# kawshik8/GAN-Image-Captioning

Measured on AMD Instinct MI355X. Metric: captions/sec (G+D train step), higher is better.
Workload: dtype bf16; 1 GPU; cfg2: adversarial G+D step, batch 64/GPU, 224x224 images, caption len 20, V=10000, E=H=512, 1-layer LSTM G, CNN-seq D (R=64,F=900), ResNet-50-shaped encoder, --conditional-gan 1; global_batch=64, caption_len=20, image_size=224, vocab=10000, conditional_gan=1, encoder=resnet50, step_impl=fused, parallelism=dp1

## Files before the change

gan-image-captioning_amd/csrc/gemm.hip:

```cpp
#include "gemm.h"
#include "conv3x3.h"
#include "conv1x1_stream.h"
#include "conv1x1_panel.h"
#include "conv1x1_pix.h"
#include "conv_stem.h"
#include "bn_fold.h"
#include "kernels.h"

#include <stdlib.h>

namespace gic {

namespace {

typedef __attribute__((address_space(3))) bf16x4 lds_bf16x4;
typedef unsigned int u32x4 __attribute__((ext_vector_type(4)));
typedef const __attribute__((address_space(1))) u32x4* gptr_u4;

__device__ __attribute__((aligned(16))) unsigned int g_zero16[4] = {0u, 0u, 0u, 0u};
typedef __attribute__((address_space(3))) void* lds_void_ptr;
typedef const __attribute__((address_space(1))) void* gbl_void_ptr;

#ifdef GIC_STAMPS
}
// ... 404 lines not shown
    for (int j = 0; j < TN; ++j) {
      const int n = bn0 + wc * (BN / 2) + j * 16 + lr;
      if (n >= N) continue;
      const float bias = (d.bias && blockIdx.y == 0) ? d.bias[n] : 0.f;
      const int mb = bm0 + wr * (BM / 2) + i * 16 + lg * 4;
      float keep4[4] = {1.f, 1.f, 1.f, 1.f};
      if constexpr (EPI == EPI_HIGHWAY) {
        if (!d.mask && d.use_philox) {
          uint32_t r0, r1, r2, r3;
          Philox::gen4(d.seed_dev ? *d.seed_dev : d.seed, d.stream, (uint64_t)(mb >> 2) * (uint64_t)N + (uint64_t)n, r0, r1, r2, r3);
          keep4[0] = Philox::u01(r0) >= d.drop_p ? 1.f : 0.f;
          keep4[1] = Philox::u01(r1) >= d.drop_p ? 1.f : 0.f;
          keep4[2] = Philox::u01(r2) >= d.drop_p ? 1.f : 0.f;
          keep4[3] = Philox::u01(r3) >= d.drop_p ? 1.f : 0.f;
        }
      }
      float st_s = 0.f, st_q = 0.f;
#pragma unroll
      for (int r = 0; r < 4; ++r) {
        const int m = mb + r;
        if (m >= M) continue;
        float v = d.alpha * acc[i][j][r] + bias;
        if constexpr (EPI == EPI_BNSTATS) {
          C[(long)m * d.ldc + n] = from_f32<TO>(v);
          st_s += v; st_q += v * v;
        } else if constexpr (EPI == EPI_PLAIN) {
          const long o = (long)m * d.ldc + n;
          if constexpr (sizeof(TO) == 4) {
            if (split) { atomicAdd((float*)&C[o], v); continue; }
          }
          if (d.accumulate) v += to_f32<TO>(C[o]);
          C[o] = from_f32<TO>(v);
        } else {
          const float x = to_f32<TI>(((const TI*)d.X)[(long)m * d.ldx + n]);
          const float sg = 1.f / (1.f + expf(-v));
          const float y = sg * fmaxf(v, 0.f) + (1.f - sg) * x;
          if (d.Hpre) d.Hpre[(long)m * d.ldh + n] = v;
          float keep = keep4[r];
          if (d.mask) keep = (float)d.mask[(long)m * d.ldmask + n];
          if (d.mask_out) d.mask_out[(long)m * d.ldmask_out + n] = (uint8_t)keep;
          C[(long)m * d.ldc + n] = from_f32<TO>(y * keep * d.keep_scale);
        }
      }
      if constexpr (EPI == EPI_BNSTATS) {
        st_s += __shfl_xor(st_s, 16, 64); st_q += __shfl_xor(st_q, 16, 64);
        st_s += __shfl_xor(st_s, 32, 64); st_q += __shfl_xor(st_q, 32, 64);
        float* st = d.stats + (long)(blockIdx.x % d.stats_nrep) * 2 * N;
        if (lg == 0) { atomicAdd(&st[n], st_s); atomicAdd(&st[N + n], st_q); }
      }
    }
  }
}

template <typename TO, int BN, int EPI, bool CONV, int NS, bool ABN = false, bool ARES = false, int AMAXK = (ARES ? 2048 : 1024)>
__global__ __launch_bounds__(512) void tile8_kernel(const GemmDesc d, const unsigned a_bytes, const unsigned b_bytes) {
  static_assert(!ARES || ABN, "the residual-on-load form extends the A-side BatchNorm");
  constexpr int BM = 128, BK = 64, NT = 512;
  constexpr int TM = 2, TN = BN / 32;
  constexpr int CA = BM * 8 / NT, CB = BN * 8 / NT;
  constexpr int NL = CA + CB + (ARES ? CA : 0);
  constexpr int A_BYTES = BM * 128, B_BYTES = BN * 128, R_BYTES = ARES ? A_BYTES : 0, STAGE = A_BYTES + B_BYTES + R_BYTES;
  constexpr int OSZ = sizeof(TO), OVE = 16 / OSZ, SC = BN * OSZ + 16;
  constexpr int EPI_BYTES = EPI == EPI_HIGHWAY ? BM * (BN + 4) * 4 : (EPI == EPI_GUMBELMAX ? 8 * BN * 4 : BM * SC + 8 * (BN / 2) * 2 * 4);
  constexpr int RING_BYTES = NS * STAGE > EPI_BYTES ? NS * STAGE : EPI_BYTES;
  constexpr int ABN_MAXK = AMAXK;
  constexpr int SMEM_BYTES = RING_BYTES + (ABN ? ABN_MAXK * 8 : 0) + (ARES ? ABN_MAXK * 8 : 0);
  constexpr unsigned OOB = 0x80000000u;
  static_assert(CB >= 1 && SMEM_BYTES <= 160 * 1024, "tile8 LDS budget");
  __shared__ __attribute__((aligned(16))) unsigned char smem[SMEM_BYTES];

  const int tid = threadIdx.x, lane = tid & 63, w = tid >> 6;
  STAMP(0);
  const int wr = w >> 1, wc = w & 1;
  const int lr = lane & 15, lg = lane >> 4;

  const int tiles_m = (d.M + BM - 1) / BM, tiles_n = (d.N + BN - 1) / BN;
  const int bid = xcd_run(blockIdx.x, gridDim.x);
  const int bm0 = (d.n_fast ? bid / tiles_n : bid % tiles_m) * BM;
  const int bn0 = (d.n_fast ? bid % tiles_n : bid / tiles_m) * BN;
  const int M = d.M, N = d.N, K = d.K;

  const __amdgpu_buffer_rsrc_t rsA = __builtin_amdgcn_make_buffer_rsrc((void*)d.A, 0, (int)a_bytes, 0x00020000);
  const __amdgpu_buffer_rsrc_t rsB = __builtin_amdgcn_make_buffer_rsrc((void*)d.B, 0, (int)b_bytes, 0x00020000);
  const __amdgpu_buffer_rsrc_t rsR = __builtin_amdgcn_make_buffer_rsrc((void*)(ARES ? d.res : d.A), 0, (int)a_bytes, 0x00020000);

  const int kc = ((tid & 7) ^ ((tid >> 4) & 7)) * 8;
  int a_off[CA], a_hi0[CA], a_wi0[CA];
  bool a_ok[CA];
  int cv_r = 0, cv_s = 0, cv_c = 0;
#pragma unroll
  for (int i = 0; i < CA; ++i) {
    const int m = bm0 + (tid >> 3) + i * 64;
    a_ok[i] = m < M;
    if constexpr (CONV) {
      const int mm = a_ok[i] ? m : 0;
      const int wo = mm % d.cWo, t = mm / d.cWo;
      const int ho = t % d.cHo, n = t / d.cHo;
      a_hi0[i] = a_ok[i] ? ho * d.cStride - d.cPad : -(1 << 28);
      a_wi0[i] = wo * d.cStride - d.cPad;
      a_off[i] = ((n * d.cH + a_hi0[i]) * d.cW + a_wi0[i]) * d.cCin;
    } else {
      a_hi0[i] = a_wi0[i] = 0;
      a_off[i] = m * (int)d.lda;
    }
  }
  if constexpr (CONV) {
    cv_c = kc % d.cCin;
    const int t = kc / d.cCin;
    cv_s = t % d.cKW;
    cv_r = t / d.cKW;
  }
  int b_off[CB];
  bool b_ok[CB];
#pragma unroll
  for (int i = 0; i < CB; ++i) {
    const int n = bn0 + (tid >> 3) + i * 64;
    b_ok[i] = n < N;
    b_off[i] = n * (int)d.ldb;
  }
  const int wbase = (tid & ~63) * 16;

  auto issue = [&](int kt, int st) {
    unsigned char* sA = smem + st * STAGE;
    unsigned char* sB = sA + A_BYTES;
    const int k = kt * BK + kc;
    const bool kok = k < K;
#pragma unroll
    for (int i = 0; i < CA; ++i) {
      unsigned voff;
      if constexpr (CONV) {
        const bool ok = (unsigned)(a_hi0[i] + cv_r) < (unsigned)d.cH & (unsigned)(a_wi0[i] + cv_s) < (unsigned)d.cW & kok;
        voff = ok ? (unsigned)(a_off[i] + (cv_r * d.cW + cv_s) * d.cCin + cv_c) * 2u : OOB;
      } else {
        voff = (a_ok[i] & kok) ? (unsigned)(a_off[i] + k) * 2u : OOB;
      }
      __builtin_amdgcn_raw_ptr_buffer_load_lds(rsA, (lds_void_ptr)(sA + i * (NT * 16) + wbase), 16, (int)voff, 0, 0, CONV ? GIC_TRUNK_NT : 0);
      if constexpr (ARES)
        __builtin_amdgcn_raw_ptr_buffer_load_lds(rsR, (lds_void_ptr)(sB + B_BYTES + i * (NT * 16) + wbase), 16, (int)voff, 0, 0, CONV ? GIC_TRUNK_NT : 0);
    }
#pragma unroll
    for (int i = 0; i < CB; ++i) {
      const unsigned voff = (b_ok[i] & kok) ? (unsigned)(b_off[i] + k) * 2u : OOB;
      __builtin_amdgcn_raw_ptr_buffer_load_lds(rsB, (lds_void_ptr)(sB + i * (NT * 16) + wbase), 16, (int)voff, 0, 0, 0);
    }
    if constexpr (CONV) {
      cv_c += BK;
      while (cv_c >= d.cCin) {
        cv_c -= d.cCin;
        if (++cv_s == d.cKW) { cv_s = 0; ++cv_r; }
      }
    }
  };

  float* coef = (float*)(smem + RING_BYTES);
  if constexpr (ABN) {
    const int Cn = CONV ? d.cCin : K;
    for (int c = tid; c < ABN_MAXK; c += NT) {
      float sc = 0.f, sh = 0.f;
      if (c < Cn) {
        float s1, s2;
        fold_replicas(d.in_stats, d.in_nrep, Cn, c, s1, s2);
        const float mean = s1 * d.in_inv_count;
        const float var = fmaxf(s2 * d.in_inv_count - mean * mean, 0.f);
        sc = d.in_gamma[c] * rsqrtf(var + 1e-5f);
        sh = d.in_beta[c] - mean * sc;
      }
      coef[2 * c] = sc; coef[2 * c + 1] = sh;
      if constexpr (ARES) {
        float rs = 1.f, rt = 0.f;
        if (d.res_stats && c < Cn) {
          float s1, s2;
          fold_replicas(d.res_stats, d.res_nrep, Cn, c, s1, s2);
          const float mean = s1 * d.res_inv_count;
          const float var = fmaxf(s2 * d.res_inv_count - mean * mean, 0.f);
          rs = d.res_gamma[c] * rsqrtf(var + 1e-5f);
          rt = d.res_beta[c] - mean * rs;
        }
        coef[2 * ABN_MAXK + 2 * c] = rs; coef[2 * ABN_MAXK + 2 * c + 1] = rt;
      }
    }
    __syncthreads();
  }
  const bool wb = ARES && d.out_wb && bn0 == 0;
  auto abn = [&](int kt, int st) {
    if constexpr (ABN) {
      const int k = kt * BK + kc;
      if (k < K) {
        const int ch = CONV ? k % d.cCin : k;
        const int tap = CONV ? k / d.cCin : 0;
        const int ts = tap % (CONV ? d.cKW : 1), tr = tap / (CONV ? d.cKW : 1);
        const float4* cp = (const float4*)(coef + 2 * ch);
        const float4 c0 = cp[0], c1 = cp[1], c2 = cp[2], c3 = cp[3];
        const float scl[8] = {c0.x, c0.z, c1.x, c1.z, c2.x, c2.z, c3.x, c3.z};
        const float sft[8] = {c0.y, c0.w, c1.y, c1.w, c2.y, c2.w, c3.y, c3.w};
        float rsc[8] = {1.f, 1.f, 1.f, 1.f, 1.f, 1.f, 1.f, 1.f}, rsf[8] = {0.f, 0.f, 0.f, 0.f, 0.f, 0.f, 0.f, 0.f};
        if constexpr (ARES) {
          const float4* rp = (const float4*)(coef + 2 * ABN_MAXK + 2 * ch);
          const float4 r0 = rp[0], r1 = rp[1], r2 = rp[2], r3 = rp[3];
          rsc[0] = r0.x; rsc[1] = r0.z; rsc[2] = r1.x; rsc[3] = r1.z; rsc[4] = r2.x; rsc[5] = r2.z; rsc[6] = r3.x; rsc[7] = r3.z;
          rsf[0] = r0.y; rsf[1] = r0.w; rsf[2] = r1.y; rsf[3] = r1.w; rsf[4] = r2.y; rsf[5] = r2.w; rsf[6] = r3.y; rsf[7] = r3.w;
        }
#pragma unroll
        for (int i = 0; i < CA; ++i) {
          const bool ok = CONV ? ((unsigned)(a_hi0[i] + tr) < (unsigned)d.cH & (unsigned)(a_wi0[i] + ts) < (unsigned)d.cW) : a_ok[i];
          if (!ok) continue;
          bf16x8* p = (bf16x8*)(smem + st * STAGE + i * (NT * 16) + tid * 16);
          bf16x8 v = *p;
          if constexpr (ARES) {
            const bf16x8 r = *(const bf16x8*)(smem + st * STAGE + A_BYTES + B_BYTES + i * (NT * 16) + tid * 16);
#pragma unroll
            for (int e = 0; e < 8; ++e) v[e] = (bf16_t)fmaxf((float)v[e] * scl[e] + sft[e] + ((float)r[e] * rsc[e] + rsf[e]), 0.f);
            if (wb) *(bf16x8*)((bf16_t*)d.out_wb + (long)a_off[i] + k) = v;
          } else {
#pragma unroll
            for (int e = 0; e < 8; ++e) v[e] = (bf16_t)fmaxf((float)v[e] * scl[e] + sft[e], 0.f);
          }
          *p = v;
        }
      }
    }
  };

  f32x4 acc[TM][TN];
#pragma unroll
  for (int i = 0; i < TM; ++i)
#pragma unroll
    for (int j = 0; j < TN; ++j) acc[i][j] = (f32x4){0.f, 0.f, 0.f, 0.f};

  auto compute = [&](int st) {
    const unsigned char* sA = smem + st * STAGE;
    const unsigned char* sB = sA + A_BYTES;
    bf16x8 fa[2][TM], fb[2][TN];
#pragma unroll
    for (int ks = 0; ks < 2; ++ks) {
#pragma unroll
      for (int t = 0; t < TM; ++t) {
        const int row = wr * 32 + t * 16 + lr;
        fa[ks][t] = *(const bf16x8*)(sA + row * 128 + (((ks * 4 + lg) ^ ((row >> 1) & 7)) << 4));
      }
#pragma unroll
      for (int t = 0; t < TN; ++t) {
        const int row = wc * (BN / 2) + t * 16 + lr;
        fb[ks][t] = *(const bf16x8*)(sB + row * 128 + (((ks * 4 + lg) ^ ((row >> 1) & 7)) << 4));
      }
    }
#pragma unroll
    for (int ks = 0; ks < 2; ++ks)
#pragma unroll
      for (int i = 0; i < TM; ++i)
#pragma unroll
        for (int j = 0; j < TN; ++j)
          acc[i][j] = __builtin_amdgcn_mfma_f32_16x16x32_bf16(fa[ks][i], fb[ks][j], acc[i][j], 0, 0, 0);
  };

  auto read_half = [&](int st, int ks, bf16x8 (&fa)[TM], bf16x8 (&fb)[TN]) {
    const unsigned char* sA = smem + st * STAGE;
    const unsigned char* sB = sA + A_BYTES;
#pragma unroll
    for (int t = 0; t < TM; ++t) {
      const int row = wr * 32 + t * 16 + lr;
      fa[t] = *(const bf16x8*)(sA + row * 128 + (((ks * 4 + lg) ^ ((row >> 1) & 7)) << 4));
    }
#pragma unroll
    for (int t = 0; t < TN; ++t) {
      const int row = wc * (BN / 2) + t * 16 + lr;
      fb[t] = *(const bf16x8*)(sB + row * 128 + (((ks * 4 + lg) ^ ((row >> 1) & 7)) << 4));
    }
  };
  auto mfma_half = [&](const bf16x8 (&fa)[TM], const bf16x8 (&fb)[TN]) {
#pragma unroll
    for (int i = 0; i < TM; ++i)
#pragma unroll
      for (int j = 0; j < TN; ++j)
        acc[i][j] = __builtin_amdgcn_mfma_f32_16x16x32_bf16(fa[i], fb[j], acc[i][j], 0, 0, 0);
  };

  const int nk = (K + BK - 1) / BK;
  STAMP(1);
  if constexpr (NS == 1) {
    for (int kt = 0; kt < nk; ++kt) {
      if (kt) __builtin_amdgcn_s_barrier();
      issue(kt, 0);
      asm volatile("s_waitcnt vmcnt(0)" ::: "memory");
      abn(kt, 0);
      __builtin_amdgcn_s_barrier();
      compute(0);
    }
  } else if constexpr (NS < 4) {
    issue(0, 0);
    int st = 0;
    for (int kt = 0; kt < nk; ++kt) {
      asm volatile("s_waitcnt vmcnt(0)" ::: "memory");
      abn(kt, st);
      __builtin_amdgcn_s_barrier();
      if (kt == 0) STAMP(2);
      if (!(DBG & 1)) issue(kt + 1, st ^ 1);
      if (!(DBG & 2)) compute(st);
      st ^= 1;
    }
  } else {
#pragma unroll
    for (int s = 0; s < NS - 1; ++s) issue(s, s);
    bf16x8 fa0[TM], fb0[TN], fa1[TM], fb1[TN];
    int st = 0, st_fill = NS - 1;
    for (int kt = 0; kt < nk; ++kt) {
      asm volatile("s_waitcnt vmcnt(%0) lgkmcnt(0)" ::"n"(NS >= 2 ? (NS - 2) * NL : 0) : "memory");
      abn(kt, st);
      __builtin_amdgcn_s_barrier();
      if (kt == 0) STAMP(2);
      if (!(DBG & 2)) {
        read_half(st, 0, fa0, fb0);
        __builtin_amdgcn_sched_barrier(0);
        if (kt > 0) mfma_half(fa1, fb1);
        __builtin_amdgcn_sched_barrier(0);
      }
      if (!(DBG & 1)) issue(kt + NS - 1, st_fill);
      if (!(DBG & 2)) {
        __builtin_amdgcn_sched_barrier(0);
        read_half(st, 1, fa1, fb1);
        __builtin_amdgcn_sched_barrier(0);
        mfma_half(fa0, fb0);
      }
      st = st == NS - 1 ? 0 : st + 1;
      st_fill = st_fill == NS - 1 ? 0 : st_fill + 1;
    }
    if (!(DBG & 2) && nk > 0) mfma_half(fa1, fb1);
  }
  asm volatile("s_waitcnt vmcnt(0)" ::: "memory");
  __syncthreads();
  STAMP(3);

  if constexpr (EPI == EPI_GUMBELMAX) {
    float* sV = (float*)smem;
    int* sI = (int*)(smem + 4 * BN * 4);
    const float eps = 1e-10f;
    const uint64_t seed = d.seed_dev ? *d.seed_dev : d.seed;
    const float T = d.gm_temperature;
#pragma unroll
    for (int j = 0; j < TN; ++j) {
      const int nl = wc * (BN / 2) + j * 16 + lr;
      const int n = bn0 + nl;
      float best = -INFINITY;
      int best_i = 0x7fffffff;
#pragma unroll
      for (int i = 0; i < TM; ++i) {
        const int m0 = bm0 + wr * 32 + i * 16 + lg * 4;
        if (m0 < M && n < N) {
          const float4 bv = *(const float4*)(d.gm_bias + m0);
          const float bia[4] = {bv.x, bv.y, bv.z, bv.w};
          float uu[4];
          if (d.gm_u) {
            const float4 uv = *(const float4*)(d.gm_u + (long)n * d.gm_ldu + m0);
            uu[0] = uv.x; uu[1] = uv.y; uu[2] = uv.z; uu[3] = uv.w;
          } else {
            uint32_t r0, r1, r2, r3;
            Philox::gen4(seed, d.stream, (uint64_t)n * (uint64_t)(M >> 2) + (uint64_t)(m0 >> 2), r0, r1, r2, r3);
            uu[0] = Philox::u01(r0); uu[1] = Philox::u01(r1); uu[2] = Philox::u01(r2); uu[3] = Philox::u01(r3);
          }
#pragma unroll
          for (int r = 0; r < 4; ++r) {
            const float g = -__logf(-__logf(uu[r] + eps) + eps);
            const float y = (acc[i][j][r] + bia[r] + g) * T;
            if (y > best) { best = y; best_i = m0 + r; }
          }
        }
      }
#pragma unroll
      for (int o = 16; o <= 32; o <<= 1) {
        const float ob = __shfl_xor(best, o, 64);
        const int oi = __shfl_xor(best_i, o, 64);
        if (ob > best || (ob == best && oi < best_i)) { best = ob; best_i = oi; }
      }
      if (lg == 0) { sV[wr * BN + nl] = best; sI[wr * BN + nl] = best_i; }
    }
    __syncthreads();
    if (tid < BN && bn0 + tid < N) {
      float best = sV[tid];
      int best_i = sI[tid];
#pragma unroll
// ... 61 lines not shown
            if (d.mask && live) k = (float)d.mask[(long)m * d.ldmask + n0 + e];
            kb |= (unsigned long long)(live ? (unsigned)k : 0u) << (8 * e);
            yv[e] = (bf16_t)(live ? y * k * d.keep_scale : 0.f);
          }
          if (d.Hpre) {
            *(float4*)(d.Hpre + (long)m * d.ldh + n0) = h0;
            *(float4*)(d.Hpre + (long)m * d.ldh + n0 + 4) = h1;
          }
          if (d.mask_out) *(unsigned long long*)(d.mask_out + (long)m * d.ldmask_out + n0) = kb;
          *(bf16x8*)((bf16_t*)C + (long)m * d.ldc + n0) = yv;
        }
      }
      STAMP(5);
      return;
    }
#pragma unroll
    for (int i = 0; i < TM; ++i) {
#pragma unroll
      for (int j = 0; j < TN; ++j) {
        const int n = bn0 + wc * (BN / 2) + j * 16 + lr;
        if (n >= N) continue;
        const float bias = d.bias ? d.bias[n] : 0.f;
        const int mb = bm0 + wr * 32 + i * 16 + lg * 4;
        float keep4[4] = {1.f, 1.f, 1.f, 1.f};
        if (!d.mask && d.use_philox) {
          uint32_t r0, r1, r2, r3;
          Philox::gen4(d.seed_dev ? *d.seed_dev : d.seed, d.stream, (uint64_t)(mb >> 2) * (uint64_t)N + (uint64_t)n, r0, r1, r2, r3);
          keep4[0] = Philox::u01(r0) >= d.drop_p ? 1.f : 0.f;
          keep4[1] = Philox::u01(r1) >= d.drop_p ? 1.f : 0.f;
          keep4[2] = Philox::u01(r2) >= d.drop_p ? 1.f : 0.f;
          keep4[3] = Philox::u01(r3) >= d.drop_p ? 1.f : 0.f;
        }
#pragma unroll
        for (int r = 0; r < 4; ++r) {
          const int m = mb + r;
          if (m >= M) continue;
          const float v = d.alpha * acc[i][j][r] + bias;
          const float x = to_f32<bf16_t>(((const bf16_t*)d.X)[(long)m * d.ldx + n]);
          const float sg = 1.f / (1.f + expf(-v));
          const float y = sg * fmaxf(v, 0.f) + (1.f - sg) * x;
          if (d.Hpre) d.Hpre[(long)m * d.ldh + n] = v;
          float keep = keep4[r];
          if (d.mask) keep = (float)d.mask[(long)m * d.ldmask + n];
          if (d.mask_out) d.mask_out[(long)m * d.ldmask_out + n] = (uint8_t)keep;
          C[(long)m * d.ldc + n] = from_f32<TO>(y * keep * d.keep_scale);
        }
      }
    }
    STAMP(5);
    return;
  }
  unsigned char* sC = smem;
  float* sStat = (float*)(smem + BM * SC);
#pragma unroll
  for (int j = 0; j < TN; ++j) {
    const int nl = wc * (BN / 2) + j * 16 + lr;
    const int n = bn0 + nl;
    const float bias = (d.bias && n < N) ? d.bias[n] : 0.f;
    float st_s = 0.f, st_q = 0.f;
#pragma unroll
    for (int i = 0; i < TM; ++i) {
#pragma unroll
      for (int r = 0; r < 4; ++r) {
        const int ml = wr * 32 + i * 16 + lg * 4 + r;
        const float v = d.alpha * acc[i][j][r] + bias;
        *(TO*)(sC + ml * SC + nl * OSZ) = from_f32<TO>(v);
        if (EPI == EPI_BNSTATS && bm0 + ml < M) { st_s += v; st_q += v * v; }
      }
    }
    if constexpr (EPI == EPI_BNSTATS) {
      st_s += __shfl_xor(st_s, 16, 64); st_q += __shfl_xor(st_q, 16, 64);
      st_s += __shfl_xor(st_s, 32, 64); st_q += __shfl_xor(st_q, 32, 64);
      if (lg == 0) { sStat[(w * (BN / 2) + j * 16 + lr) * 2] = st_s; sStat[(w * (BN / 2) + j * 16 + lr) * 2 + 1] = st_q; }
    }
  }
  __syncthreads();
  STAMP(4);
  if constexpr (EPI == EPI_BNSTATS) {
    if (tid < BN) {
      const int cwc = tid / (BN / 2), cl = tid % (BN / 2), n = bn0 + tid;
      if (n < N) {
        float s0 = 0.f, q0 = 0.f;
#pragma unroll
        for (int r = 0; r < 4; ++r) {
          s0 += sStat[((r * 2 + cwc) * (BN / 2) + cl) * 2];
          q0 += sStat[((r * 2 + cwc) * (BN / 2) + cl) * 2 + 1];
        }
        float* stp = d.stats + (long)(blockIdx.x % d.stats_nrep) * 2 * N;
        atomicAdd(&stp[n], s0);
        atomicAdd(&stp[N + n], q0);
      }
    }
  }
  constexpr int CPR = BN / OVE;
  for (int c = tid; c < BM * CPR; c += NT) {
    const int ml = c / CPR, cc = c % CPR;
    const int m = bm0 + ml, n = bn0 + cc * OVE;
    if (m < M && n < N) {
      u32x4 v = *(const u32x4*)(sC + ml * SC + cc * 16);
      if (d.accumulate) {
        const u32x4 o = *(const u32x4*)(C + (long)m * d.ldc + n);
        TO* pv = (TO*)&v;
        const TO* po = (const TO*)&o;
#pragma unroll
        for (int e = 0; e < OVE; ++e) pv[e] = from_f32<TO>(to_f32<TO>(pv[e]) + to_f32<TO>(po[e]));
      }
      *(u32x4*)(C + (long)m * d.ldc + n) = v;
    }
  }
  STAMP(5);
}

template <typename TO, int EPI, bool CONV>
bool try_tile8(const GemmDesc& d_in, hipStream_t stream) {
  static const bool off = getenv("GIC_NO_TILE8") != nullptr;
  GemmDesc d = d_in;
  constexpr int OVE = 16 / (int)sizeof(TO);
  if (off || d.M < 128) return false;
  if (EPI != EPI_HIGHWAY && ((d.N % OVE) || (d.ldc % OVE) || (((uintptr_t)d.C) & 15))) return false;
  if (EPI == EPI_HIGHWAY && d.in_dtype != DT_BF16) return false;
  if (!CONV && ((long)cdiv(d.M, 128) * cdiv(d.N, 64) < 128 || d.K < 256)) return false;
  const long a_elems = CONV ? (long)(d.M / (d.cHo * d.cWo)) * d.cH * d.cW * d.cCin : (long)(d.M - 1) * d.lda + d.K;
  const long b_elems = (long)(d.N - 1) * d.ldb + d.K;
  if (a_elems * 2 >= (1l << 31) || b_elems * 2 >= (1l << 31)) return false;
  const long big_tiles = (long)cdiv(d.M, 128) * cdiv(d.N, 128);
  static const int big_min = [] { const char* e = getenv("GIC_TILE8_BIG_MIN"); return e ? atoi(e) : 160; }();
  static const int ns2_tiles = [] { const char* e = getenv("GIC_TILE8_NS2_TILES"); return e ? atoi(e) : 256; }();
  static const int min_nk = [] { const char* e = getenv("GIC_TILE8_MIN_NK"); return e ? atoi(e) : 1; }();
  if (cdiv(d.K, 64) < min_nk) return false;
  const unsigned ab = (unsigned)(a_elems * 2), bb = (unsigned)(b_elems * 2);
  d.n_fast = xcd_share_a(2 * (a_elems < (long)d.M * d.K ? a_elems : (long)d.M * d.K), 2l * d.N * d.K, cdiv(d.N, d.N >= 128 ? 128 : 64));
  if constexpr (EPI == EPI_BNSTATS && CONV) {
    if (d.in_stats && d.res) {
      if (d.cKH != 1 || d.cKW != 1 || d.cStride != 1 || d.cPad != 0 || d.cCin % 8 || d.cCin > 2048 || !d.in_gamma || !d.in_beta ||
          d.in_inv_count <= 0.f || (d.res_stats && (!d.res_gamma || !d.res_beta || d.res_inv_count <= 0.f)))
        return false;
      const bool n128 = d.N >= 128;
      const long tiles = n128 ? big_tiles : (long)cdiv(d.M, 128) * cdiv(d.N, 64);
      const dim3 grid((unsigned)tiles), block(512);
      static const int res_ns = [] { const char* e = getenv("GIC_TILE8_RES_NS"); return e ? atoi(e) : 1; }();
      if (d.cCin <= 512) {
        if (res_ns == 1) {
          if (n128) hipLaunchKernelGGL((tile8_kernel<TO, 128, EPI, CONV, 1, true, true, 512>), grid, block, 0, stream, d, ab, bb);
          else hipLaunchKernelGGL((tile8_kernel<TO, 64, EPI, CONV, 1, true, true, 512>), grid, block, 0, stream, d, ab, bb);
        } else {
          if (n128) hipLaunchKernelGGL((tile8_kernel<TO, 128, EPI, CONV, 2, true, true, 512>), grid, block, 0, stream, d, ab, bb);
          else hipLaunchKernelGGL((tile8_kernel<TO, 64, EPI, CONV, 2, true, true, 512>), grid, block, 0, stream, d, ab, bb);
        }
      } else {
        if (res_ns == 1) {
          if (n128) hipLaunchKernelGGL((tile8_kernel<TO, 128, EPI, CONV, 1, true, true, 2048>), grid, block, 0, stream, d, ab, bb);
          else hipLaunchKernelGGL((tile8_kernel<TO, 64, EPI, CONV, 1, true, true, 2048>), grid, block, 0, stream, d, ab, bb);
        } else {
          if (n128) hipLaunchKernelGGL((tile8_kernel<TO, 128, EPI, CONV, 2, true, true, 2048>), grid, block, 0, stream, d, ab, bb);
          else hipLaunchKernelGGL((tile8_kernel<TO, 64, EPI, CONV, 2, true, true, 2048>), grid, block, 0, stream, d, ab, bb);
        }
      }
      return true;
    }
    if (d.in_stats) {
      if (d.cCin % 8 || d.cCin > 1024 || !d.in_gamma || !d.in_beta || d.in_inv_count <= 0.f) return false;
      const int nk = cdiv(d.K, 64);
      const bool n128 = d.N >= 128 && big_tiles >= big_min;
      const long tiles = n128 ? big_tiles : (long)cdiv(d.M, 128) * cdiv(d.N, 64);
      const dim3 grid((unsigned)tiles), block(512);
      if (nk <= 4 && tiles > 512) {
        if (n128) hipLaunchKernelGGL((tile8_kernel<TO, 128, EPI, CONV, 1, true>), grid, block, 0, stream, d, ab, bb);
        else hipLaunchKernelGGL((tile8_kernel<TO, 64, EPI, CONV, 1, true>), grid, block, 0, stream, d, ab, bb);
      } else if (tiles > 256) {
        if (n128) hipLaunchKernelGGL((tile8_kernel<TO, 128, EPI, CONV, 2, true>), grid, block, 0, stream, d, ab, bb);
        else hipLaunchKernelGGL((tile8_kernel<TO, 64, EPI, CONV, 2, true>), grid, block, 0, stream, d, ab, bb);
      } else {
        if (n128) hipLaunchKernelGGL((tile8_kernel<TO, 128, EPI, CONV, 4, true>), grid, block, 0, stream, d, ab, bb);
        else hipLaunchKernelGGL((tile8_kernel<TO, 64, EPI, CONV, 4, true>), grid, block, 0, stream, d, ab, bb);
      }
      return true;
    }
  }
  static const int ns1_nk = [] { const char* e = getenv("GIC_TILE8_NS1_NK"); return e ? atoi(e) : 4; }();
  const int nk8 = cdiv(d.K, 64);
  if (EPI != EPI_HIGHWAY && nk8 <= ns1_nk && (d.N >= 128 ? big_tiles : (long)cdiv(d.M, 128) * cdiv(d.N, 64)) > 512) {
    if (d.N >= 128) hipLaunchKernelGGL((tile8_kernel<TO, 128, EPI, CONV, 1>), dim3((unsigned)big_tiles), dim3(512), 0, stream, d, ab, bb);
    else hipLaunchKernelGGL((tile8_kernel<TO, 64, EPI, CONV, 1>), dim3((unsigned)(cdiv(d.M, 128) * cdiv(d.N, 64))), dim3(512), 0, stream, d, ab, bb);
    return true;
  }
  if (d.N >= 128 && big_tiles >= big_min) {
    if (big_tiles > ns2_tiles) hipLaunchKernelGGL((tile8_kernel<TO, 128, EPI, CONV, 2>), dim3((unsigned)big_tiles), dim3(512), 0, stream, d, ab, bb);
    else hipLaunchKernelGGL((tile8_kernel<TO, 128, EPI, CONV, 4>), dim3((unsigned)big_tiles), dim3(512), 0, stream, d, ab, bb);
  } else {
    const long tiles = (long)cdiv(d.M, 128) * cdiv(d.N, 64);
    if (tiles > ns2_tiles) hipLaunchKernelGGL((tile8_kernel<TO, 64, EPI, CONV, 2>), dim3((unsigned)tiles), dim3(512), 0, stream, d, ab, bb);
    else hipLaunchKernelGGL((tile8_kernel<TO, 64, EPI, CONV, 4>), dim3((unsigned)tiles), dim3(512), 0, stream, d, ab, bb);
  }
  return true;
}


__global__ void zero2d_kernel(float* __restrict__ C, long ldc, int M, int N) {
  const long total = (long)M * N;
  for (long i = (long)blockIdx.x * blockDim.x + threadIdx.x; i < total; i += (long)gridDim.x * blockDim.x)
    C[(i / N) * ldc + (i % N)] = 0.f;
}

template <typename TI, typename TO, bool AKC, bool BKC, int BM, int BN, bool VEC, int EPI, bool CONV = false>
int launch(const GemmDesc& d, hipStream_t stream) {
  constexpr int BK = 128 / (int)sizeof(TI);
  const int tiles = cdiv(d.M, BM) * cdiv(d.N, BN);
  const int nk = cdiv(d.K, BK);
  int splits = 1;
  if (EPI == EPI_PLAIN && sizeof(TI) == 2 && sizeof(TO) == 4 && !d.no_split) {
    if (tiles < 24 && nk >= 8) {
      splits = 256 / tiles;
      if (splits > nk / 2) splits = nk / 2;
      if (splits > 16) splits = 16;
    } else if (tiles <= 192 && nk >= 32) {
      splits = 512 / tiles;
      if (splits > nk / 8) splits = nk / 8;
      if (splits > 16) splits = 16;
    } else if (!AKC && !BKC && tiles <= 192 && nk >= 16) {
      splits = 512 / tiles;
      if (splits > nk / 4) splits = nk / 4;
    } else if (tiles <= 320 && nk >= 64) {
      splits = 768 / tiles;
    }
    if (splits < 1) splits = 1;
    if (det_mode()) splits = (d.accumulate || splits < 2) ? 1 : 2;
  }
  int per = cdiv(nk, splits);
  splits = cdiv(nk, per);
  if (splits > 1 && !d.accumulate && !d.c_zeroed) {
    const long total = (long)d.M * d.N;
    const int g = (int)((total + 255) / 256 > 1024 ? 1024 : (total + 255) / 256);
    hipLaunchKernelGGL(zero2d_kernel, dim3(g), dim3(256), 0, stream, (float*)d.C, d.ldc, d.M, d.N);
  }
  constexpr bool CAN_PIPE = AKC && BKC && VEC;
  static const bool no_pipe = getenv("GIC_GEMM_NO_PIPE") != nullptr;
  const bool pipe = CAN_PIPE && per >= 6 && (long)tiles * splits <= 2 * 256 + 8 && !no_pipe;
  if constexpr (CAN_PIPE) {
    if (pipe) {
      hipLaunchKernelGGL((gemm_kernel<TI, TO, AKC, BKC, BM, BN, VEC, EPI, CONV, true>), dim3(tiles, splits), dim3(256), 0, stream, d, per);
      GIC_CHECK_LAUNCH("gemm");
      return GIC_OK;
    }
  }
  hipLaunchKernelGGL((gemm_kernel<TI, TO, AKC, BKC, BM, BN, VEC, EPI, CONV, false>), dim3(tiles, splits), dim3(256), 0, stream, d, per);
  GIC_CHECK_LAUNCH("gemm");
  return GIC_OK;
}

int big_tile_min() {
  static const int v = [] { const char* e = getenv("GIC_GEMM_BIG_MIN"); return e ? atoi(e) : 192; }();
  return v;
}

template <typename TI, typename TO, bool AKC, bool BKC, int EPI>
int pick_tile(const GemmDesc& d, bool vec, hipStream_t stream) {
  const long big_tiles = (long)cdiv(d.M, 128) * cdiv(d.N, 128);
  const bool big = big_tiles >= big_tile_min() && d.M >= 128 && d.N >= 128;
  if (big) {
    return vec ? launch<TI, TO, AKC, BKC, 128, 128, true, EPI>(d, stream)
               : launch<TI, TO, AKC, BKC, 128, 128, false, EPI>(d, stream);
  }
  return vec ? launch<TI, TO, AKC, BKC, 64, 64, true, EPI>(d, stream)
             : launch<TI, TO, AKC, BKC, 64, 64, false, EPI>(d, stream);
}

template <typename TI, typename TO, int EPI>
int pick_layout(const GemmDesc& d, bool vec, hipStream_t stream) {
  if constexpr (sizeof(TI) == 2) {
    if (d.a_kc && d.b_kc && vec && try_tile8<TO, EPI, false>(d, stream)) { GIC_CHECK_LAUNCH("gemm tile8"); return GIC_OK; }
  }
  if (d.a_kc && d.b_kc) return pick_tile<TI, TO, true, true, EPI>(d, vec, stream);
  if constexpr (EPI == EPI_PLAIN) {
    if (d.a_kc && !d.b_kc) return pick_tile<TI, TO, true, false, EPI>(d, vec, stream);
    if (!d.a_kc && !d.b_kc) return pick_tile<TI, TO, false, false, EPI>(d, vec, stream);
  }
  set_last_error("gemm: unsupported layout a_kc=%d b_kc=%d epi=%d", d.a_kc, d.b_kc, d.epi);
  return GIC_ERR_UNSUPPORTED;
}

template <typename TI, typename TO, int EPI>
int pick_conv(const GemmDesc& d, hipStream_t stream) {
  if constexpr (sizeof(TI) == 2 && sizeof(TO) == 2 && EPI == EPI_BNSTATS) {
    if (try_conv_stem(d, stream)) { GIC_CHECK_LAUNCH("conv stem"); return GIC_OK; }
    if (try_conv3x3_patch(d, stream)) { GIC_CHECK_LAUNCH("conv3x3 patch"); return GIC_OK; }
    if (try_conv1x1_stream(d, stream)) { GIC_CHECK_LAUNCH("conv1x1 stream"); return GIC_OK; }
    if (d.stats_only) return GIC_ERR_UNSUPPORTED;
    if (try_conv1x1_pix(d, stream)) { GIC_CHECK_LAUNCH("conv1x1 pix"); return GIC_OK; }
    if (try_conv1x1_panel(d, stream)) { GIC_CHECK_LAUNCH("conv1x1 panel"); return GIC_OK; }
    if (d.in_stats && d.cKH * d.cKW > 1) return GIC_ERR_UNSUPPORTED;
  }
  if constexpr (sizeof(TI) == 2) {
    if (try_tile8<TO, EPI, true>(d, stream)) { GIC_CHECK_LAUNCH("conv tile8"); return GIC_OK; }
  }
  if (d.in_stats) return GIC_ERR_UNSUPPORTED;
  const long big_tiles = (long)cdiv(d.M, 128) * cdiv(d.N, 128);
  if (big_tiles >= big_tile_min() && d.N >= 128) return launch<TI, TO, true, true, 128, 128, true, EPI, true>(d, stream);
  return launch<TI, TO, true, true, 64, 64, true, EPI, true>(d, stream);
}

template <typename TI, typename TO>
int pick_epi(const GemmDesc& d, bool vec, hipStream_t stream) {
  if (d.conv) {
    if (!vec || !d.a_kc || !d.b_kc) { set_last_error("gemm: convolution needs 16-B aligned NHWC / KRSC operands"); return GIC_ERR_UNSUPPORTED; }
    if constexpr (sizeof(TI) == sizeof(TO)) {
      if (d.epi == EPI_BNSTATS) return pick_conv<TI, TO, EPI_BNSTATS>(d, stream);
      if (d.epi == EPI_PLAIN) return pick_conv<TI, TO, EPI_PLAIN>(d, stream);
    }
    set_last_error("gemm: unsupported convolution epilogue / dtype");
    return GIC_ERR_UNSUPPORTED;
  }
  if (d.epi == EPI_PLAIN) return pick_layout<TI, TO, EPI_PLAIN>(d, vec, stream);
  if (d.epi == EPI_HIGHWAY) return pick_layout<TI, TO, EPI_HIGHWAY>(d, vec, stream);
  set_last_error("gemm: unknown epilogue %d", d.epi);
  return GIC_ERR_UNSUPPORTED;
}

bool aligned16(const void* p) { return (((uintptr_t)p) & 15) == 0; }

}

int gemm_gumbelmax(const GemmDesc& d0, hipStream_t stream) {
  GemmDesc d = d0;
  static const bool off = getenv("GIC_NO_TILE8") != nullptr || getenv("GIC_NO_FUSED_GUMBELMAX") != nullptr;
  GIC_CHECK_ARG(d.A && d.B && d.gm_rowkey && d.gm_bias, "gemm_gumbelmax: null operand");
  if (off || d.in_dtype != DT_BF16 || !d.a_kc || !d.b_kc || d.M < 128 || d.M % 4 || d.K % 8 || d.lda % 8 || d.ldb % 8 || !aligned16(d.A) ||
      !aligned16(d.B) || !aligned16(d.gm_bias) || (d.gm_u && (!aligned16(d.gm_u) || d.gm_ldu % 4)) || !(d.gm_temperature > 0.f))
    return GIC_ERR_UNSUPPORTED;
  const long a_elems = (long)(d.M - 1) * d.lda + d.K, b_elems = (long)(d.N - 1) * d.ldb + d.K;
  const long tiles = (long)cdiv(d.M, 128) * cdiv(d.N, 128);
  if (a_elems * 2 >= (1l << 31) || b_elems * 2 >= (1l << 31) || d.N < 128 || tiles < 160) return GIC_ERR_UNSUPPORTED;
  d.epi = EPI_GUMBELMAX;
  d.n_fast = xcd_share_a(2l * d.M * d.K, 2l * d.N * d.K, cdiv(d.N, 128));
  const unsigned ab = (unsigned)(a_elems * 2), bb = (unsigned)(b_elems * 2);
  if (tiles > 256) hipLaunchKernelGGL((tile8_kernel<float, 128, EPI_GUMBELMAX, false, 2>), dim3((unsigned)tiles), dim3(512), 0, stream, d, ab, bb);
  else hipLaunchKernelGGL((tile8_kernel<float, 128, EPI_GUMBELMAX, false, 4>), dim3((unsigned)tiles), dim3(512), 0, stream, d, ab, bb);
  GIC_CHECK_LAUNCH("gemm gumbelmax");
  return GIC_OK;
}

int gemm(const GemmDesc& d0, hipStream_t stream) {
  GemmDesc d = d0;
#ifdef GIC_STAMPS
  { const char* e = getenv("GIC_GEMM_DBG"); if (e) d.dbg = atoi(e); }
#endif
  GIC_CHECK_ARG(d.A && d.B && d.C, "gemm: null operand");
  GIC_CHECK_ARG(d.M >= 0 && d.N >= 0 && d.K >= 0, "gemm: negative dim");
  if (d.M == 0 || d.N == 0) return GIC_OK;
  {
    static const bool log = getenv("GIC_GEMM_LOG") != nullptr;
    if (log && !d.conv)
      fprintf(stderr, "[gemm] M=%d N=%d K=%d a_kc=%d b_kc=%d in=%d out=%d epi=%d acc=%d\n", d.M, d.N, d.K, d.a_kc, d.b_kc, d.in_dtype, d.out_dtype, d.epi,
              d.accumulate);
  }
  if (d.epi == EPI_HIGHWAY) GIC_CHECK_ARG(d.X, "gemm: highway epilogue needs X");
  const int sz = dtype_size(d.in_dtype);
  const int ve = 16 / sz;
  bool vec = aligned16(d.A) && aligned16(d.B) && (d.lda % ve == 0) && (d.ldb % ve == 0);
  if (d.conv) {
    const bool chunk_ok = (d.cCin % ve == 0) || (d.cPad == 0 && ve % d.cCin == 0 && (d.cKW * d.cCin) % ve == 0);
    GIC_CHECK_ARG(chunk_ok && d.K == d.cKH * d.cKW * d.cCin && d.K % ve == 0, "gemm: conv needs Cin %% %d == 0 (or a pre-padded NHWC4 stem) and K = KH*KW*Cin", ve);
    GIC_CHECK_ARG(d.epi != EPI_BNSTATS || d.stats, "gemm: EPI_BNSTATS needs a stats buffer");
    vec = aligned16(d.A) && aligned16(d.B) && (d.ldb % ve == 0);
  }
  if (d.a_kc || d.b_kc) vec = vec && (d.K % ve == 0);
  if (d.in_dtype == DT_F32 && d.out_dtype == DT_F32) return pick_epi<float, float>(d, vec, stream);
  if (d.in_dtype == DT_BF16 && d.out_dtype == DT_F32) return pick_epi<bf16_t, float>(d, vec, stream);
  if (d.in_dtype == DT_BF16 && d.out_dtype == DT_BF16) return pick_epi<bf16_t, bf16_t>(d, vec, stream);
  set_last_error("gemm: unsupported dtypes in=%d out=%d", d.in_dtype, d.out_dtype);
  return GIC_ERR_UNSUPPORTED;
}

}
#ifdef GIC_STAMPS
extern "C" int gic_debug_stamps(unsigned long long* out) {
  return (int)hipMemcpyFromSymbol(out, HIP_SYMBOL(gic::g_stamp), sizeof(unsigned long long) * 32);
}
#endif
```

Before: 26640 captions/s.

## Extend tile8 GEMM to transposed operands via LDS transpose reads and split-K

Adds a transposed-operand path to the tile8 MFMA kernel. B (and optionally A) are loaded with their K dimension outermost, then fed to the MFMAs through ds_read_tr16 transpose reads from a swizzled LDS layout. For fp32 outputs on small tile counts, K is split across blocks, partials are combined with atomics, and the split index is spread across XCDs. This routes backward-pass weight and input gradient GEMMs (NN/TN layouts) away from the older generic gemm_kernel. The cost is extra atomics, a zeroing pass, and a scalar tail fix for partial rows, with nondeterminism unless deterministic mode is on.

```diff
diff --git a/gan-image-captioning_amd/csrc/gemm.hip b/gan-image-captioning_amd/csrc/gemm.hip
--- a/gan-image-captioning_amd/csrc/gemm.hip
+++ b/gan-image-captioning_amd/csrc/gemm.hip
@@ -480,9 +480,27 @@
   }
 }
 
-template <typename TO, int BN, int EPI, bool CONV, int NS, bool ABN = false, bool ARES = false, int AMAXK = (ARES ? 2048 : 1024)>
+template <int R>
+__device__ __forceinline__ int tr_swz(const int kk) {
+  return R == 128 ? (((kk & 3) << 2) | ((kk >> 2) & 3)) : ((kk & 2) | ((kk >> 1) & 4));
+}
+template <int R>
+__device__ __forceinline__ bf16x8 tr_frag(const unsigned char* s, const int r0, const int ks, const int lr, const int lg) {
+  const int q = lr >> 2, p = lr & 3;
+  const int kk = ks * 32 + lg * 8 + q, ch = (r0 >> 3) + (p >> 1);
+  const unsigned char* p0 = s + kk * (2 * R) + 16 * (ch ^ tr_swz<R>(kk)) + 8 * (p & 1);
+  const unsigned char* p1 = s + (kk + 4) * (2 * R) + 16 * (ch ^ tr_swz<R>(kk + 4)) + 8 * (p & 1);
+  const bf16x4 t0 = __builtin_amdgcn_ds_read_tr16_b64_v4bf16((lds_bf16x4*)p0);
+  const bf16x4 t1 = __builtin_amdgcn_ds_read_tr16_b64_v4bf16((lds_bf16x4*)p1);
+  return __builtin_shufflevector(t0, t1, 0, 1, 2, 3, 4, 5, 6, 7);
+}
+
+template <typename TO, int BN, int EPI, bool CONV, int NS, bool ABN = false, bool ARES = false, int AMAXK = (ARES ? 2048 : 1024),
+          bool AKC = true, bool BKC = true>
 __global__ __launch_bounds__(512) void tile8_kernel(const GemmDesc d, const unsigned a_bytes, const unsigned b_bytes) {
   static_assert(!ARES || ABN, "the residual-on-load form extends the A-side BatchNorm");
+  constexpr bool TR = !AKC || !BKC;
+  static_assert(!TR || (EPI == EPI_PLAIN && !CONV && !ABN && NS >= 2), "transposed operands: plain products on a ring only");
   constexpr int BM = 128, BK = 64, NT = 512;
   constexpr int TM = 2, TN = BN / 32;
   constexpr int CA = BM * 8 / NT, CB = BN * 8 / NT;
@@ -503,7 +521,15 @@
   const int lr = lane & 15, lg = lane >> 4;
 
   const int tiles_m = (d.M + BM - 1) / BM, tiles_n = (d.N + BN - 1) / BN;
-  const int bid = xcd_run(blockIdx.x, gridDim.x);
+  int bid, split = blockIdx.y;
+  if (TR && (gridDim.y & 7) == 0) {
+    const int lin = blockIdx.x + gridDim.x * blockIdx.y;
+    const int j = lin >> 3;
+    split = (lin & 7) * (gridDim.y >> 3) + j / gridDim.x;
+    bid = j % gridDim.x;
+  } else {
+    bid = xcd_run(blockIdx.x, gridDim.x);
+  }
   const int bm0 = (d.n_fast ? bid / tiles_n : bid % tiles_m) * BM;
   const int bn0 = (d.n_fast ? bid % tiles_n : bid / tiles_m) * BN;
   const int M = d.M, N = d.N, K = d.K;
@@ -548,15 +574,50 @@
   }
   const int wbase = (tid & ~63) * 16;
 
+  const int nk = (K + BK - 1) / BK;
+  const int per = TR ? (nk + (int)gridDim.y - 1) / (int)gridDim.y : nk;
+  const int kt0 = TR ? split * per : 0;
+  const int nkl = TR ? max(0, min(nk, kt0 + per) - kt0) : nk;
+  const int kend = TR ? min(K, (kt0 + nkl) * BK) : K;
+
+  constexpr int CPR_A = BM / 8, CPR_B = BN / 8;
+  int ta_kk[CA], tb_kk[CB];
+  int ta_row = 0, tb_row = 0, ta_kend = kend, tb_kend = kend;
+  bool ta_ok = false, tb_ok = false, ta_tail = false, tb_tail = false;
+  if constexpr (!AKC) {
+#pragma unroll
+    for (int i = 0; i < CA; ++i) ta_kk[i] = (tid + i * NT) / CPR_A;
+    ta_row = bm0 + 8 * ((tid % CPR_A) ^ tr_swz<BM>(ta_kk[0]));
+    ta_ok = ta_row < M;
+    ta_tail = ta_row + 8 > M;
+    if (ta_tail) ta_kend = min(kend, K - 1);
+#pragma unroll
+    for (int i = 0; i < CA; ++i) a_off[i] = ta_kk[i] * (int)d.lda + ta_row;
+  }
+  if constexpr (!BKC) {
+#pragma unroll
+    for (int i = 0; i < CB; ++i) tb_kk[i] = (tid + i * NT) / CPR_B;
+    tb_row = bn0 + 8 * ((tid % CPR_B) ^ tr_swz<BN>(tb_kk[0]));
+    tb_ok = tb_row < N;
+    tb_tail = tb_row + 8 > N;
+    if (tb_tail) tb_kend = min(kend, K - 1);
+#pragma unroll
+    for (int i = 0; i < CB; ++i) b_off[i] = tb_kk[i] * (int)d.ldb + tb_row;
+  }
+
   auto issue = [&](int kt, int st) {
     unsigned char* sA = smem + st * STAGE;
     unsigned char* sB = sA + A_BYTES;
+    kt += kt0;
     const int k = kt * BK + kc;
-    const bool kok = k < K;
+    const bool kok = k < kend;
 #pragma unroll
     for (int i = 0; i < CA; ++i) {
       unsigned voff;
-      if constexpr (CONV) {
+      if constexpr (!AKC) {
+        const bool ok = ta_ok & (kt * BK + ta_kk[i] < ta_kend);
+        voff = ok ? (unsigned)(a_off[i] + kt * BK * (int)d.lda) * 2u : OOB;
+      } else if constexpr (CONV) {
         const bool ok = (unsigned)(a_hi0[i] + cv_r) < (unsigned)d.cH & (unsigned)(a_wi0[i] + cv_s) < (unsigned)d.cW & kok;
         voff = ok ? (unsigned)(a_off[i] + (cv_r * d.cW + cv_s) * d.cCin + cv_c) * 2u : OOB;
       } else {
@@ -568,7 +629,13 @@
     }
 #pragma unroll
     for (int i = 0; i < CB; ++i) {
-      const unsigned voff = (b_ok[i] & kok) ? (unsigned)(b_off[i] + k) * 2u : OOB;
+      unsigned voff;
+      if constexpr (!BKC) {
+        const bool ok = tb_ok & (kt * BK + tb_kk[i] < tb_kend);
+        voff = ok ? (unsigned)(b_off[i] + kt * BK * (int)d.ldb) * 2u : OOB;
+      } else {
+        voff = (b_ok[i] & kok) ? (unsigned)(b_off[i] + k) * 2u : OOB;
+      }
       __builtin_amdgcn_raw_ptr_buffer_load_lds(rsB, (lds_void_ptr)(sB + i * (NT * 16) + wbase), 16, (int)voff, 0, 0, 0);
     }
     if constexpr (CONV) {
@@ -609,6 +676,42 @@
     }
     __syncthreads();
   }
+  auto tail_fix = [&](int kt, int st) {
+    if constexpr (TR) {
+      const int kk = K - 1 - (kt0 + kt) * BK;
+      bool done = false;
+      if constexpr (!AKC) {
+        if (ta_ok & ta_tail & ((unsigned)kk < (unsigned)BK)) {
+#pragma unroll
+          for (int i = 0; i < CA; ++i) {
+            if (ta_kk[i] != kk) continue;
+            const bf16_t* src = (const bf16_t*)d.A + (long)(K - 1) * d.lda + ta_row;
+            bf16x8 v;
+#pragma unroll
+            for (int e = 0; e < 8; ++e) v[e] = ta_row + e < M ? src[e] : (bf16_t)0.f;
+            *(bf16x8*)(smem + st * STAGE + i * (NT * 16) + tid * 16) = v;
+            done = true;
+          }
+        }
+      }
+      if constexpr (!BKC) {
+        if (tb_ok & tb_tail & ((unsigned)kk < (unsigned)BK)) {
+#pragma unroll
+          for (int i = 0; i < CB; ++i) {
+            if (tb_kk[i] != kk) continue;
+            const bf16_t* src = (const bf16_t*)d.B + (long)(K - 1) * d.ldb + tb_row;
+            bf16x8 v;
+#pragma unroll
+            for (int e = 0; e < 8; ++e) v[e] = tb_row + e < N ? src[e] : (bf16_t)0.f;
+            *(bf16x8*)(smem + st * STAGE + A_BYTES + i * (NT * 16) + tid * 16) = v;
+            done = true;
+          }
+        }
+      }
+      if (done) asm volatile("s_waitcnt lgkmcnt(0)" ::: "memory");
+    }
+  };
+
   const bool wb = ARES && d.out_wb && bn0 == 0;
   auto abn = [&](int kt, int st) {
     if constexpr (ABN) {
@@ -664,12 +767,14 @@
 #pragma unroll
       for (int t = 0; t < TM; ++t) {
         const int row = wr * 32 + t * 16 + lr;
-        fa[ks][t] = *(const bf16x8*)(sA + row * 128 + (((ks * 4 + lg) ^ ((row >> 1) & 7)) << 4));
+        if constexpr (!AKC) fa[ks][t] = tr_frag<BM>(sA, wr * 32 + t * 16, ks, lr, lg);
+        else fa[ks][t] = *(const bf16x8*)(sA + row * 128 + (((ks * 4 + lg) ^ ((row >> 1) & 7)) << 4));
       }
 #pragma unroll
       for (int t = 0; t < TN; ++t) {
         const int row = wc * (BN / 2) + t * 16 + lr;
-        fb[ks][t] = *(const bf16x8*)(sB + row * 128 + (((ks * 4 + lg) ^ ((row >> 1) & 7)) << 4));
+        if constexpr (!BKC) fb[ks][t] = tr_frag<BN>(sB, wc * (BN / 2) + t * 16, ks, lr, lg);
+        else fb[ks][t] = *(const bf16x8*)(sB + row * 128 + (((ks * 4 + lg) ^ ((row >> 1) & 7)) << 4));
       }
     }
 #pragma unroll
@@ -687,12 +792,14 @@
 #pragma unroll
     for (int t = 0; t < TM; ++t) {
       const int row = wr * 32 + t * 16 + lr;
-      fa[t] = *(const bf16x8*)(sA + row * 128 + (((ks * 4 + lg) ^ ((row >> 1) & 7)) << 4));
+      if constexpr (!AKC) fa[t] = tr_frag<BM>(sA, wr * 32 + t * 16, ks, lr, lg);
+      else fa[t] = *(const bf16x8*)(sA + row * 128 + (((ks * 4 + lg) ^ ((row >> 1) & 7)) << 4));
     }
 #pragma unroll
     for (int t = 0; t < TN; ++t) {
       const int row = wc * (BN / 2) + t * 16 + lr;
-      fb[t] = *(const bf16x8*)(sB + row * 128 + (((ks * 4 + lg) ^ ((row >> 1) & 7)) << 4));
+      if constexpr (!BKC) fb[t] = tr_frag<BN>(sB, wc * (BN / 2) + t * 16, ks, lr, lg);
+      else fb[t] = *(const bf16x8*)(sB + row * 128 + (((ks * 4 + lg) ^ ((row >> 1) & 7)) << 4));
     }
   };
   auto mfma_half = [&](const bf16x8 (&fa)[TM], const bf16x8 (&fb)[TN]) {
@@ -703,10 +810,9 @@
         acc[i][j] = __builtin_amdgcn_mfma_f32_16x16x32_bf16(fa[i], fb[j], acc[i][j], 0, 0, 0);
   };
 
-  const int nk = (K + BK - 1) / BK;
   STAMP(1);
   if constexpr (NS == 1) {
-    for (int kt = 0; kt < nk; ++kt) {
+    for (int kt = 0; kt < nkl; ++kt) {
       if (kt) __builtin_amdgcn_s_barrier();
       issue(kt, 0);
       asm volatile("s_waitcnt vmcnt(0)" ::: "memory");
@@ -717,9 +823,10 @@
   } else if constexpr (NS < 4) {
     issue(0, 0);
     int st = 0;
-    for (int kt = 0; kt < nk; ++kt) {
+    for (int kt = 0; kt < nkl; ++kt) {
       asm volatile("s_waitcnt vmcnt(0)" ::: "memory");
       abn(kt, st);
+      tail_fix(kt, st);
       __builtin_amdgcn_s_barrier();
       if (kt == 0) STAMP(2);
       if (!(DBG & 1)) issue(kt + 1, st ^ 1);
@@ -731,9 +838,10 @@
     for (int s = 0; s < NS - 1; ++s) issue(s, s);
     bf16x8 fa0[TM], fb0[TN], fa1[TM], fb1[TN];
     int st = 0, st_fill = NS - 1;
-    for (int kt = 0; kt < nk; ++kt) {
+    for (int kt = 0; kt < nkl; ++kt) {
       asm volatile("s_waitcnt vmcnt(%0) lgkmcnt(0)" ::"n"(NS >= 2 ? (NS - 2) * NL : 0) : "memory");
       abn(kt, st);
+      tail_fix(kt, st);
       __builtin_amdgcn_s_barrier();
       if (kt == 0) STAMP(2);
       if (!(DBG & 2)) {
@@ -752,7 +860,7 @@
       st = st == NS - 1 ? 0 : st + 1;
       st_fill = st_fill == NS - 1 ? 0 : st_fill + 1;
     }
-    if (!(DBG & 2) && nk > 0) mfma_half(fa1, fb1);
+    if (!(DBG & 2) && nkl > 0) mfma_half(fa1, fb1);
   }
   asm volatile("s_waitcnt vmcnt(0)" ::: "memory");
   __syncthreads();
@@ -920,11 +1028,12 @@
   }
   unsigned char* sC = smem;
   float* sStat = (float*)(smem + BM * SC);
+  const bool split_c = TR && gridDim.y > 1;
 #pragma unroll
   for (int j = 0; j < TN; ++j) {
     const int nl = wc * (BN / 2) + j * 16 + lr;
     const int n = bn0 + nl;
-    const float bias = (d.bias && n < N) ? d.bias[n] : 0.f;
+    const float bias = (d.bias && n < N && (!split_c || split == 0)) ? d.bias[n] : 0.f;
     float st_s = 0.f, st_q = 0.f;
 #pragma unroll
     for (int i = 0; i < TM; ++i) {
@@ -958,6 +1067,17 @@
         atomicAdd(&stp[n], s0);
         atomicAdd(&stp[N + n], q0);
       }
+    }
+  }
+  if constexpr (TR && sizeof(TO) == 4) {
+    if (split_c) {
+      for (int e = tid; e < BM * BN; e += NT) {
+        const int ml = e / BN, nl = e % BN;
+        const int m = bm0 + ml, n = bn0 + nl;
+        if (m < M && n < N) atomicAdd((float*)C + (long)m * d.ldc + n, *(const float*)(sC + ml * SC + nl * 4));
+      }
+      STAMP(5);
+      return;
     }
   }
   constexpr int CPR = BN / OVE;
@@ -978,6 +1098,9 @@
   }
   STAMP(5);
 }
+
+struct GemmPick { const char* kernel; int bm, bn, ns, splits; };
+GemmPick g_pick = {"-", 0, 0, 0, 0};
 
 template <typename TO, int EPI, bool CONV>
 bool try_tile8(const GemmDesc& d_in, hipStream_t stream) {
@@ -1048,15 +1171,18 @@
   static const int ns1_nk = [] { const char* e = getenv("GIC_TILE8_NS1_NK"); return e ? atoi(e) : 4; }();
   const int nk8 = cdiv(d.K, 64);
   if (EPI != EPI_HIGHWAY && nk8 <= ns1_nk && (d.N >= 128 ? big_tiles : (long)cdiv(d.M, 128) * cdiv(d.N, 64)) > 512) {
+    g_pick = {"tile8", 128, d.N >= 128 ? 128 : 64, 1, 1};
     if (d.N >= 128) hipLaunchKernelGGL((tile8_kernel<TO, 128, EPI, CONV, 1>), dim3((unsigned)big_tiles), dim3(512), 0, stream, d, ab, bb);
     else hipLaunchKernelGGL((tile8_kernel<TO, 64, EPI, CONV, 1>), dim3((unsigned)(cdiv(d.M, 128) * cdiv(d.N, 64))), dim3(512), 0, stream, d, ab, bb);
     return true;
   }
   if (d.N >= 128 && big_tiles >= big_min) {
+    g_pick = {"tile8", 128, 128, big_tiles > ns2_tiles ? 2 : 4, 1};
     if (big_tiles > ns2_tiles) hipLaunchKernelGGL((tile8_kernel<TO, 128, EPI, CONV, 2>), dim3((unsigned)big_tiles), dim3(512), 0, stream, d, ab, bb);
     else hipLaunchKernelGGL((tile8_kernel<TO, 128, EPI, CONV, 4>), dim3((unsigned)big_tiles), dim3(512), 0, stream, d, ab, bb);
   } else {
     const long tiles = (long)cdiv(d.M, 128) * cdiv(d.N, 64);
+    g_pick = {"tile8", 128, 64, tiles > ns2_tiles ? 2 : 4, 1};
     if (tiles > ns2_tiles) hipLaunchKernelGGL((tile8_kernel<TO, 64, EPI, CONV, 2>), dim3((unsigned)tiles), dim3(512), 0, stream, d, ab, bb);
     else hipLaunchKernelGGL((tile8_kernel<TO, 64, EPI, CONV, 4>), dim3((unsigned)tiles), dim3(512), 0, stream, d, ab, bb);
   }
@@ -1104,6 +1230,7 @@
   constexpr bool CAN_PIPE = AKC && BKC && VEC;
   static const bool no_pipe = getenv("GIC_GEMM_NO_PIPE") != nullptr;
   const bool pipe = CAN_PIPE && per >= 6 && (long)tiles * splits <= 2 * 256 + 8 && !no_pipe;
+  g_pick = {"gemm_kernel", BM, BN, pipe ? 3 : 2, splits};
   if constexpr (CAN_PIPE) {
     if (pipe) {
       hipLaunchKernelGGL((gemm_kernel<TI, TO, AKC, BKC, BM, BN, VEC, EPI, CONV, true>), dim3(tiles, splits), dim3(256), 0, stream, d, per);
@@ -1114,6 +1241,53 @@
   hipLaunchKernelGGL((gemm_kernel<TI, TO, AKC, BKC, BM, BN, VEC, EPI, CONV, false>), dim3(tiles, splits), dim3(256), 0, stream, d, per);
   GIC_CHECK_LAUNCH("gemm");
   return GIC_OK;
+}
+
+template <typename TO, bool AKC>
+bool try_tile8_t(const GemmDesc& d_in, hipStream_t stream) {
+  static const bool off = getenv("GIC_NO_TILE8") != nullptr || getenv("GIC_NO_TILE8_T") != nullptr;
+  static const int target = [] { const char* e = getenv("GIC_TILE8_T_BLOCKS"); return e ? atoi(e) : 256; }();
+  static const bool xcd_split = getenv("GIC_TILE8_T_NO_XCD_SPLIT") == nullptr;
+  GemmDesc d = d_in;
+  constexpr int OVE = 16 / (int)sizeof(TO);
+  if (off || d.M < 128 || d.K < 256) return false;
+  if ((d.N % OVE) || (d.ldc % OVE) || (((uintptr_t)d.C) & 15) || (((uintptr_t)d.A) & 15) || (((uintptr_t)d.B) & 15)) return false;
+  if ((d.lda % 8) || (d.ldb % 8) || (AKC && d.K % 8) || (!AKC && d.lda < d.M) || d.ldb < d.N) return false;
+  const long a_elems = AKC ? (long)(d.M - 1) * d.lda + d.K : (long)(d.K - 1) * d.lda + d.M;
+  const long b_elems = (long)(d.K - 1) * d.ldb + d.N;
+  if (a_elems * 2 >= (1l << 30) || b_elems * 2 >= (1l << 30)) return false;
+  const int bn = d.N >= 128 ? 128 : 64;
+  const long tiles = (long)cdiv(d.M, 128) * cdiv(d.N, bn);
+  const int nk = cdiv(d.K, 64);
+  int splits = 1;
+  if (sizeof(TO) == 4 && !d.no_split && tiles < target) {
+    splits = (int)(target / tiles);
+    if (splits > nk / 8) splits = nk / 8;
+    if (splits > 16) splits = 16;
+    if (xcd_split && nk >= 64 && tiles <= 80) splits = 8;
+    if (splits < 1) splits = 1;
+    if (det_mode()) splits = (d.accumulate || splits < 2) ? 1 : 2;
+  }
+  const int per = cdiv(nk, splits);
+  splits = cdiv(nk, per);
+  if (splits == 1 && tiles < 128) return false;
+  if (splits > 1 && !d.accumulate && !d.c_zeroed) {
+    const long total = (long)d.M * d.N;
+    const int g = (int)((total + 255) / 256 > 1024 ? 1024 : (total + 255) / 256);
+    hipLaunchKernelGGL(zero2d_kernel, dim3(g), dim3(256), 0, stream, (float*)d.C, d.ldc, d.M, d.N);
+  }
+  d.n_fast = xcd_share_a(2 * (a_elems < (long)d.M * d.K ? a_elems : (long)d.M * d.K), 2l * d.N * d.K, cdiv(d.N, bn));
+  const unsigned ab = (unsigned)(a_elems * 2), bb = (unsigned)(b_elems * 2);
+  const bool ns2 = bn == 128 && tiles * splits > 256;
+  const dim3 grid((unsigned)tiles, (unsigned)splits), block(512);
+  g_pick = {AKC ? "tile8 NN" : "tile8 TN", 128, bn, ns2 ? 2 : 4, splits};
+  if (bn == 128) {
+    if (ns2) hipLaunchKernelGGL((tile8_kernel<TO, 128, EPI_PLAIN, false, 2, false, false, 1024, AKC, false>), grid, block, 0, stream, d, ab, bb);
+    else hipLaunchKernelGGL((tile8_kernel<TO, 128, EPI_PLAIN, false, 4, false, false, 1024, AKC, false>), grid, block, 0, stream, d, ab, bb);
+  } else {
+    hipLaunchKernelGGL((tile8_kernel<TO, 64, EPI_PLAIN, false, 4, false, false, 1024, AKC, false>), grid, block, 0, stream, d, ab, bb);
+  }
+  return true;
 }
 
 int big_tile_min() {
@@ -1139,6 +1313,12 @@
     if (d.a_kc && d.b_kc && vec && try_tile8<TO, EPI, false>(d, stream)) { GIC_CHECK_LAUNCH("gemm tile8"); return GIC_OK; }
   }
   if (d.a_kc && d.b_kc) return pick_tile<TI, TO, true, true, EPI>(d, vec, stream);
+  if constexpr (EPI == EPI_PLAIN && sizeof(TI) == 2) {
+    if (vec && !d.b_kc && (d.a_kc ? try_tile8_t<TO, true>(d, stream) : try_tile8_t<TO, false>(d, stream))) {
+      GIC_CHECK_LAUNCH("gemm tile8 transposed");
+      return GIC_OK;
+    }
+  }
   if constexpr (EPI == EPI_PLAIN) {
     if (d.a_kc && !d.b_kc) return pick_tile<TI, TO, true, false, EPI>(d, vec, stream);
     if (!d.a_kc && !d.b_kc) return pick_tile<TI, TO, false, false, EPI>(d, vec, stream);
@@ -1215,12 +1395,6 @@
   GIC_CHECK_ARG(d.A && d.B && d.C, "gemm: null operand");
   GIC_CHECK_ARG(d.M >= 0 && d.N >= 0 && d.K >= 0, "gemm: negative dim");
   if (d.M == 0 || d.N == 0) return GIC_OK;
-  {
-    static const bool log = getenv("GIC_GEMM_LOG") != nullptr;
-    if (log && !d.conv)
-      fprintf(stderr, "[gemm] M=%d N=%d K=%d a_kc=%d b_kc=%d in=%d out=%d epi=%d acc=%d\n", d.M, d.N, d.K, d.a_kc, d.b_kc, d.in_dtype, d.out_dtype, d.epi,
-              d.accumulate);
-  }
   if (d.epi == EPI_HIGHWAY) GIC_CHECK_ARG(d.X, "gemm: highway epilogue needs X");
   const int sz = dtype_size(d.in_dtype);
   const int ve = 16 / sz;
@@ -1232,11 +1406,22 @@
     vec = aligned16(d.A) && aligned16(d.B) && (d.ldb % ve == 0);
   }
   if (d.a_kc || d.b_kc) vec = vec && (d.K % ve == 0);
-  if (d.in_dtype == DT_F32 && d.out_dtype == DT_F32) return pick_epi<float, float>(d, vec, stream);
-  if (d.in_dtype == DT_BF16 && d.out_dtype == DT_F32) return pick_epi<bf16_t, float>(d, vec, stream);
-  if (d.in_dtype == DT_BF16 && d.out_dtype == DT_BF16) return pick_epi<bf16_t, bf16_t>(d, vec, stream);
-  set_last_error("gemm: unsupported dtypes in=%d out=%d", d.in_dtype, d.out_dtype);
-  return GIC_ERR_UNSUPPORTED;
+  g_pick = {"-", 0, 0, 0, 0};
+  int rc;
+  if (d.in_dtype == DT_F32 && d.out_dtype == DT_F32) rc = pick_epi<float, float>(d, vec, stream);
+  else if (d.in_dtype == DT_BF16 && d.out_dtype == DT_F32) rc = pick_epi<bf16_t, float>(d, vec, stream);
+  else if (d.in_dtype == DT_BF16 && d.out_dtype == DT_BF16) rc = pick_epi<bf16_t, bf16_t>(d, vec, stream);
+  else {
+    set_last_error("gemm: unsupported dtypes in=%d out=%d", d.in_dtype, d.out_dtype);
+    return GIC_ERR_UNSUPPORTED;
+  }
+  {
+    static const bool log = getenv("GIC_GEMM_LOG") != nullptr;
+    if (log && !d.conv)
+      fprintf(stderr, "[gemm] M=%d N=%d K=%d a_kc=%d b_kc=%d in=%d out=%d epi=%d acc=%d -> %s %dx%d ns=%d splits=%d\n", d.M, d.N, d.K, d.a_kc,
+              d.b_kc, d.in_dtype, d.out_dtype, d.epi, d.accumulate, g_pick.kernel, g_pick.bm, g_pick.bn, g_pick.ns, g_pick.splits);
+  }
+  return rc;
 }
 
 }
```

Result: no change. 26650 captions/s, median of 6 (+0.0%).
